# YangChenApril/AMContrast3D

Measured on AMD Instinct MI355X. Metric: train-step points/sec (fwd+bwd) on 24k-pt S3DIS clouds, higher is better.
Workload: dtype f32; 1 GPU; PointNeXt-S + AMContrast3D-AA, S3DIS-shaped 24000-pt voxelised (0.04 m) clouds, batch 8/GPU, fwd + CE/contrast loss + bwd + clip + AdamW; global_batch=8, points=24000, parallelism=dp1, launch=hipGraph replay, batches_per_joint_fps_launch=4, geometry_queue_cus=176, feature_graph_segments=1, collectives=none, update=captured in the feature graph

## Files before the change

amcontrast3d_amd/_lib.py:

```python
import ctypes
import os
import subprocess

_CSRC = os.path.join(os.path.dirname(os.path.abspath(__file__)), "csrc")
_SO = os.environ.get("AMC3D_LIB") or os.path.join(_CSRC, "libamc3d_hip.so")

_vp, _i, _f, _sz, _l = ctypes.c_void_p, ctypes.c_int, ctypes.c_float, ctypes.c_size_t, ctypes.c_long
_ll = ctypes.c_longlong

SIGNATURES = {
    "amc3d_version": (ctypes.c_char_p, []),
    "amc3d_last_error": (ctypes.c_char_p, []),
    "amc3d_stream_create_dedicated": (_i, [ctypes.POINTER(ctypes.c_void_p)]),
    "amc3d_stream_create_masked": (_i, [_vp, _i, _i]),
    "amc3d_reserve_scratch": (_i, [_i, _vp, _vp]),
    "amc3d_stream_destroy": (_i, [_vp]),
    "amc3d_grid_search_workspace_bytes": (_sz, [_i, _i, _i]),
    "amc3d_grid_search_pays": (_i, [_i, _i, _i]),
    "amc3d_ball_query": (_i, [_i, _i, _i, _f, _i, _vp, _vp, _vp, _vp, _sz, _vp]),
    "amc3d_group_points": (_i, [_i, _i, _i, _i, _i, _vp, _vp, _vp, _vp]),
    "amc3d_group_points_grad": (_i, [_i, _i, _i, _i, _i, _vp, _vp, _vp, _vp, _sz, _vp]),
    "amc3d_gather_points": (_i, [_i, _i, _i, _i, _vp, _vp, _vp, _vp]),
    "amc3d_gather_points_grad": (_i, [_i, _i, _i, _i, _vp, _vp, _vp, _vp]),
    "amc3d_fps_workspace_bytes": (_sz, [_i, _i]),
    "amc3d_furthest_point_sampling": (_i, [_i, _i, _i, _vp, _vp, _vp, _vp, _sz, _vp]),
    "amc3d_three_nn": (_i, [_i, _i, _i, _vp, _vp, _vp, _vp, _vp, _sz, _vp]),
    "amc3d_three_interpolate": (_i, [_i, _i, _i, _i, _vp, _vp, _vp, _vp, _vp]),
    "amc3d_three_interpolate_add": (_i, [_i, _i, _i, _i, _vp, _vp, _vp, _vp, _vp, _vp]),
    "amc3d_three_interpolate_grad": (_i, [_i, _i, _i, _i, _vp, _vp, _vp, _vp, _vp, _sz, _vp]),
    "amc3d_three_interpolate_grad_route": (_i, [_i, _i, _i, _i, ctypes.POINTER(_i), ctypes.POINTER(_i)]),
    "amc3d_three_interpolate_grad_write": (_i, [_i, _i, _i, _i, _vp, _vp, _vp, _vp, _vp]),
    "amc3d_three_interpolate_grad_lds": (_i, [_i, _i, _i, _i, _i, _i, _i, _vp, _vp, _vp, _vp, _vp]),
    "amc3d_knnquery_workspace_bytes": (_sz, [_i, _i, _i, _i]),
    "amc3d_knnquery_uses_grid": (_i, [_i, _i, _i, _i]),
    "amc3d_knnquery": (_i, [_i, _i, _i, _i, _vp, _vp, _vp, _vp, _vp, _vp, _vp, _sz, _i, _vp]),
    "amc3d_knn_batch_workspace_bytes": (_sz, [_i, _i, _i, _i]),
    "amc3d_knn_batch": (_i, [_i, _i, _i, _i, _i, _vp, _vp, _vp, _vp, _i, _vp, _sz, _i, _vp]),
    "amc3d_knn_group_dp": (_i, [_i, _i, _i, _i, _vp, _vp, _vp, _i, _i, _vp, _vp, _vp]),
    "amc3d_pointops_ballquery": (_i, [_i, _f, _i, _i, _i, _vp, _vp, _vp, _vp, _vp, _vp]),
    "amc3d_pointops_furthestsampling": (_i, [_i, _i, _i, _vp, _vp, _vp, _vp, _vp, _vp]),
    "amc3d_pointops_grouping_forward": (_i, [_i, _i, _i, _i, _vp, _vp, _vp, _vp]),
    "amc3d_pointops_grouping_backward": (_i, [_i, _i, _i, _i, _vp, _vp, _vp, _vp]),
    "amc3d_pointops_interpolation_forward": (_i, [_i, _i, _i, _i, _i, _vp, _vp, _vp, _vp, _vp]),
    "amc3d_pointops_interpolation_backward": (_i, [_i, _i, _i, _i, _vp, _vp, _vp, _vp, _vp]),
    "amc3d_pointops_subtraction_forward": (_i, [_i, _i, _i, _vp, _vp, _vp, _vp, _vp]),
    "amc3d_pointops_subtraction_backward": (_i, [_i, _i, _i, _vp, _vp, _vp, _vp, _vp]),
    "amc3d_pointops_aggregation_forward": (_i, [_i, _i, _i, _i, _i, _vp, _vp, _vp, _vp, _vp, _vp]),
    "amc3d_pointops_aggregation_backward": (_i, [_i, _i, _i, _i, _vp, _vp, _vp, _vp, _vp, _vp, _vp, _vp, _vp]),
    "amc3d_pointops_scatter_csr": (_i, [_i, _i, _i, _i, _i, _vp, _vp, _vp, _vp, _vp, _vp]),
    "amc3d_vote_labels": (_i, [_i, _i, _i, _vp, _vp, _vp, _vp]),
    "amc3d_posmask": (_i, [_i, _i, _i, _vp, _vp, _vp, _vp]),
    "amc3d_ambiguity_workspace_bytes": (_sz, [_i]),
    "amc3d_ambiguity": (_i, [_i, _i, _i, _i, _f, _vp, _vp, _vp, _vp, _vp, _sz, _vp]),
    "amc3d_contrast_csr_workspace_bytes": (_sz, [_i]),
    "amc3d_contrast_csr": (_i, [_i, _i, _i, _vp, _vp, _vp, _vp, _sz, _vp]),
    "amc3d_contrast_backward_csr_supported": (_i, [_i]),
    "amc3d_contrast_backward_rows_supported": (_i, [_i]),
    "amc3d_contrast_backward_csr": (_i, [_i, _i, _i, _i, _vp, _vp, _vp, _vp, _vp, _vp, _vp, _f, _f, _f, _vp, _vp, _vp, _vp,
                                         _vp, _vp]),
    "amc3d_contrast_mutual_workspace_bytes": (_sz, [_i]),
    "amc3d_contrast_mutual": (_i, [_i, _i, _i, _vp, _vp, _vp, _vp, _vp, _vp, _sz, _vp]),
    "amc3d_contrast_backward_mutual_workspace_bytes": (_sz, [_i]),
    "amc3d_contrast_backward_mutual": (_i, [_i, _i, _i, _i, _vp, _vp, _vp, _vp, _vp, _vp, _vp, _f, _f, _f, _vp, _vp, _vp, _vp, _vp, _sz,
                                            _vp, _vp]),
    "amc3d_contrast_stages_forward_cm": (_i, [_i, _vp, _f, _f, _f, _f, _vp, _vp]),
    "amc3d_contrast_stages_backward_cm_workspace_bytes": (_sz, [_i, _vp]),
    "amc3d_contrast_stages_backward_cm": (_i, [_i, _vp, _f, _f, _f, _f, _vp, _vp, _sz, _vp]),
    "amc3d_contrast_variant_forward": (_i, [_i, _i, _i, _i, _vp, _vp, _vp, _vp, _vp, _i, _i, _i, _i, _f, _f, _f, _vp, _vp, _vp, _vp,
                                            _vp, _vp]),
    "amc3d_contrast_variant_backward": (_i, [_i, _i, _i, _i, _vp, _vp, _vp, _vp, _vp, _vp, _vp, _i, _i, _i, _i, _f, _f, _f, _vp, _vp,
                                             _vp, _vp, _vp, _vp]),
    "amc3d_adamw_chunk": (_i, []),
    "amc3d_adamw_step": (_i, [_vp, _vp, _i, ctypes.c_double, ctypes.c_double, _f, _f, _vp, _vp, _vp]),
    "amc3d_select_anchors_ints": (_sz, [_i]),
    "amc3d_select_anchors": (_i, [_i, _vp, _vp, _sz, _vp]),
    "amc3d_contrast_forward": (_i, [_i, _i, _i, _i, _vp, _vp, _vp, _vp, _vp, _f, _f, _f, _vp, _vp, _vp, _vp, _vp, _vp, _vp]),
# ... 112 lines not shown
    "amc3d_grouped_conv_bn_backward_csr": (_i, [_i] * 6 + [_vp, _i] + [_vp] * 16 + [_i, _vp, _vp, _vp, _sz, _vp]),
    "amc3d_grouped_conv_bn_backward_csr_strided": (_i, [_i] * 6 + [_vp, _i] + [_vp] * 6 + [_l] + [_vp] * 8 + [_l] + [_vp] * 2 + [_i, _vp, _vp, _vp, _sz, _vp]),
    "amc3d_group_csr_dp": (_i, [_i, _i, _i, _vp, _vp, _vp, _vp]),
    "amc3d_sa_tail_supported": (_i, [_i, _i, _i]),
    "amc3d_sa_tail_pays": (_i, [_i, _i]),
    "amc3d_sa_tail_workspace_bytes": (_sz, [_i, _i, _i, _i]),
    "amc3d_sa_tail_forward": (_i, [_i, _i, _i, _i, _i] + [_vp] * 8 + [_f, _f, _i] + [_vp] * 10 + [_sz, _vp]),
    "amc3d_sa_tail_backward": (_i, [_i, _i, _i, _i, _i] + [_vp] * 10 + [_i, _vp, _vp, _vp, _vp, _i] + [_vp] * 5 + [_sz, _vp]),
    "amc3d_bn_workspace_bytes": (_sz, [_i]),
    "amc3d_bn_stats": (_i, [_i, _i, _l, _f, _vp, _vp, _vp, _vp, _vp, _sz, _vp]),
    "amc3d_bn_forward": (_i, [_i, _i, _l, _i, _i, _f, _f, _vp, _vp, _vp, _vp, _vp, _vp, _vp, _vp, _vp, _vp, _vp, _vp, _sz, _vp]),
    "amc3d_bn_update_running": (_i, [_i, _f, _vp, _vp, _vp, _vp, _vp, _vp]),
    "amc3d_bn_act": (_i, [_i, _i, _l, _i, _vp, _vp, _vp, _vp, _vp, _vp, _vp]),
    "amc3d_bn_max": (_i, [_i, _i, _i, _i, _i, _vp, _vp, _vp, _vp, _vp, _vp, _vp, _vp]),
    "amc3d_bn_backward": (_i, [_i, _i, _l, _i, _i, _vp, _vp, _vp, _vp, _vp, _vp, _vp, _vp, _vp, _vp, _vp, _sz, _vp]),
    "amc3d_bn_sums": (_i, [_i, _i, _l, _vp, _vp, _vp, _sz, _vp]),
    "amc3d_bn_forward_synced": (_i, [_i, _i, _l, _i, _i, _f, _f, _vp, _vp, _vp, _vp, _vp, _vp, _vp, _vp, _vp, _vp, _vp, _vp, _vp]),
    "amc3d_bn_backward_sums": (_i, [_i, _i, _l, _i, _i, _vp, _vp, _vp, _vp, _vp, _vp, _vp, _vp, _vp, _vp, _vp, _sz, _vp]),
    "amc3d_bn_backward_synced": (_i, [_i, _i, _l, _i, _i, _vp, _vp, _vp, _vp, _vp, _vp, _vp, _vp, _vp, _vp, _vp]),
}


CONTRAST_MAX_STAGES = 8


class ContrastStageDesc(ctypes.Structure):
    _fields_ = ([(n, _i) for n in ("b", "C", "n", "k", "nbr_stride")]
                + [(n, _vp) for n in ("f_cm", "nbr", "posmask", "a", "sel", "mutual", "rev", "norm", "unit", "stats", "loss_pt",
                                      "mean_cnt", "rec", "grad_cm")])


def build(force=False):
    cmd = ["make", "-C", _CSRC, "-j8"] + (["-B"] if force else [])
    proc = subprocess.run(cmd, stdout=subprocess.PIPE, stderr=subprocess.STDOUT, text=True)
    if proc.returncode != 0:
        raise RuntimeError("building libamc3d_hip.so failed:\n" + proc.stdout)
    return _SO


_lib = None


def load():
    global _lib
    if _lib is not None:
        return _lib
# ... 18 lines not shown
```

amcontrast3d_amd/csrc/knn.hip:

```cpp

#include "common.h"

namespace amc {

constexpr int KNN_TILE = 1024;
constexpr int KNN_WAVES = 16;
constexpr int KNN_MAXK = 100;

__device__ __forceinline__ void reheap(float *dist, int *idx, int k)
{
    int root = 0;
    int child = 1;
    while (child < k) {
        if (child + 1 < k && dist[child + 1] > dist[child]) child++;
        if (dist[root] > dist[child]) return;
        const float tf = dist[root]; dist[root] = dist[child]; dist[child] = tf;
        const int ti = idx[root]; idx[root] = idx[child]; idx[child] = ti;
        root = child;
        child = root * 2 + 1;
    }
}

__global__ __launch_bounds__(KNN_WAVES * 64) void knn_exact_kernel(
    int m, int nsample, int nbatch, const float *__restrict__ xyz, const float *__restrict__ new_xyz,
// ... 932 lines not shown
        }
#ifdef AMC_KNN_DIAG
        if (threadIdx.x == 0)
            printf("replay q=%d T=%d |S|=%d steps=%d survsteps=%d surv=%d acc=%d  prefix_clk=%lld surv_clk=%lld\n", pt, end, ns,
                   n_steps, n_survsteps, n_surv, n_acc, (long long)(clock64() - t_a), t_surv);
#endif
        if (wave == 0) {
            float root = s_root;
            for (int r = nsample; r < ns; ++r) {
                const float cd = s_rd[r];
                if (cd < root) {
                    lh_replace_root(hp, nsample, lane, cd, s_ri[r]);
                    root = lh_root(hp);
                }
            }
            for (int i = nsample - 1; i > 0; i--) {
                const float d0 = lh_root(hp), di = __int_as_float(__builtin_amdgcn_readlane(__float_as_int(hp.d), i));
                const int j0 = __builtin_amdgcn_readlane(hp.id, 0), ji = __builtin_amdgcn_readlane(hp.id, i);
                if (lane == i) { hp.d = d0; hp.id = j0; }
                lh_replace_root(hp, i, lane, di, ji);
            }
            if (lane < nsample) {
                idx[(size_t)pt * nsample + lane] = hp.id;
                dist2[(size_t)pt * nsample + lane] = hp.d;
            }
        }
    }
}

static int kg_build(const KnnWorkspace &w, char *base, int n, int m, int nbatch, const float *xyz, const float *new_xyz,
                    const int *offset, const int *new_offset, int ksample, int sub, float hscale, float fixed_h,
                    hipStream_t stream)
{
    GridParams *gp = (GridParams *)(base + w.params);
    int *bbox = (int *)(base + w.bbox);
    float *samples = (float *)(base + w.samples);
    int *fb_count = (int *)(base + w.fb_count);
    int *cell_start = (int *)(base + w.cell_start);
    int *cursor = (int *)(base + w.cursor);
    float4 *sorted = (float4 *)(base + w.sorted);
    const size_t cells = (size_t)knn_cell_cap(n) + 1;
    if (int st = fill_i32(cell_start, 0, (size_t)(cursor - cell_start) + cells, stream)) return st;
    hipLaunchKernelGGL(kg_init_kernel, dim3(1), dim3(64), 0, stream, bbox, fb_count);
    hipLaunchKernelGGL(kg_bbox_kernel, dim3(min(div_up(n, 256), 64)), dim3(256), 0, stream, n, xyz, bbox);
    if (!(fixed_h > 0.f))
        hipLaunchKernelGGL(kg_sample_kernel, dim3(KG_SAMPLES), dim3(1024), 0, stream, m, ksample, nbatch, sub, xyz, new_xyz,
                           offset, new_offset, samples);
    hipLaunchKernelGGL(kg_params_kernel, dim3(1), dim3(64), 0, stream, n, nbatch, hscale, fixed_h, bbox, samples, gp);
    hipLaunchKernelGGL(kg_count_kernel, dim3(div_up(n, 256)), dim3(256), 0, stream, n, nbatch, xyz, offset, gp,
// ... 260 lines not shown
    if (nsample <= KGG_MAXK) {
        constexpr int per_wg = 4 * (64 / KGG_MAXK);
        hipLaunchKernelGGL(kg_query_group_kernel<KGG_MAXK>, dim3(min(div_up(m, per_wg), 256 * 32)), dim3(256), 0, stream, m,
                           nsample, nbatch, self, new_xyz, offset, new_offset, gp, cell_start, sorted, idx, dist2, fb_list,
                           fb_count);
    } else {
        hipLaunchKernelGGL(kg_query_kernel, dim3(min(div_up(m, 4), 256 * 32)), dim3(256), 0, stream, m, nsample, nbatch, self,
                           new_xyz, offset, new_offset, gp, cell_start, sorted, idx, dist2, fb_list, fb_count);
    }
    hipLaunchKernelGGL(knn_exact_list_kernel, dim3(256), dim3(1024), 0, stream, nsample, nbatch, xyz, new_xyz, offset,
                       new_offset, idx, dist2, (const int *)fb_list, (const int *)fb_count, (const GridParams *)gp,
                       (const int *)cell_start, (const float4 *)sorted);
    return launch_status("amc3d_knnquery");
}

AMC_API int amc3d_knnquery(int m, int nsample, int n, int nbatch, const float *xyz, const float *new_xyz,
                           const int *offset, const int *new_offset, int *idx, float *dist2, void *workspace,
                           size_t workspace_bytes, int reuse_grid, void *stream_)
{
    return knn_search(m, nsample, n, nbatch, xyz, new_xyz, offset, new_offset, idx, dist2, workspace, workspace_bytes,
                      reuse_grid, stream_);
}

namespace amc {

constexpr int KB_QT = 64;

struct KnnBatchWorkspace {
    size_t grid_bytes, off_s, off_q, idx, dist2, total;
};

static KnnBatchWorkspace knn_batch_layout(int b, int n, int m, int ksearch)
{
    KnnBatchWorkspace w;
    w.grid_bytes = knn_layout(b * n, b * m).total;
    w.off_s = w.grid_bytes;
    w.off_q = align256(w.off_s + (size_t)b * 4);
    w.idx = align256(w.off_q + (size_t)b * 4);
    w.dist2 = align256(w.idx + (size_t)b * m * ksearch * 4);
    w.total = align256(w.dist2 + (size_t)b * m * ksearch * 4);
    return w;
}

__global__ __launch_bounds__(256) void knn_batch_epilogue_kernel(int n, int m, int ksearch, int dilation, int kout,
                                                                 const int *__restrict__ raw_idx,
                                                                 const float *__restrict__ raw_d2, int *__restrict__ idx,
// ... 73 lines not shown
```

amcontrast3d_amd/csrc/loss.hip:

```cpp
#include "common.h"

#include <type_traits>
#include <utility>

namespace amc {

__global__ __launch_bounds__(256) void vote_labels_kernel(int m, int kr, int ncls, const int *__restrict__ labels0,
                                                          const int *__restrict__ nbr, int *__restrict__ out)
{
    const int lane = threadIdx.x & 63;
    const int q = blockIdx.x * 4 + (threadIdx.x >> 6);
    if (q >= m) return;
    int c0 = -1, c1 = -1;
    if (lane < kr) c0 = labels0[nbr[(size_t)q * kr + lane]];
    if (lane + 64 < kr) c1 = labels0[nbr[(size_t)q * kr + lane + 64]];
    int best = -1, bestc = 0;
    for (int c = 0; c < ncls; ++c) {
        const int cnt = (int)__popcll(__ballot(c0 == c)) + (int)__popcll(__ballot(c1 == c));
        if (cnt > best) { best = cnt; bestc = c; }
    }
    if (lane == 0) out[q] = bestc;
}

__global__ void posmask_kernel(int m, int k, int nbr_stride, const int *__restrict__ labels,
// ... 10 lines not shown
                                                              const unsigned char *__restrict__ posmask,
                                                              const int *__restrict__ nbr, int *__restrict__ n_pos,
                                                              float *__restrict__ d_pos, float *__restrict__ d_neg,
                                                              int *__restrict__ max_npos)
{
    const int i = blockIdx.x * blockDim.x + threadIdx.x;
    int np = 0;
    if (i < m) {
        const float px = p[(size_t)i * 3], py = p[(size_t)i * 3 + 1], pz = p[(size_t)i * 3 + 2];
        const float ss = __fadd_rn(__fadd_rn(__fmul_rn(px, px), __fmul_rn(py, py)), __fmul_rn(pz, pz));
        float dp = 0.f, dn = 0.f;
        for (int j = 0; j < k; ++j) {
            const int nb = nbr[(size_t)i * nbr_stride + j];
            const float qx = p[(size_t)nb * 3], qy = p[(size_t)nb * 3 + 1], qz = p[(size_t)nb * 3 + 2];
            const float dot = __fadd_rn(__fadd_rn(__fmul_rn(px, qx), __fmul_rn(py, qy)), __fmul_rn(pz, qz));
            const float sd = __fadd_rn(__fadd_rn(__fmul_rn(qx, qx), __fmul_rn(qy, qy)), __fmul_rn(qz, qz));
            float dd = __fadd_rn(__fadd_rn(__fmul_rn(-2.f, dot), ss), sd);
            if (mode == 3) dd = sqrtf(__fadd_rn(fabsf(dd), 1e-12f));
            const bool pos = posmask[(size_t)i * k + j] != 0;
            np += pos ? 1 : 0;
            dp = __fadd_rn(dp, pos ? dd : 0.f);
            dn = __fadd_rn(dn, pos ? 0.f : dd);
        }
        n_pos[i] = np;
        d_pos[i] = mode == 1 ? 5.f : dp;
        d_neg[i] = mode == 1 ? 5.f : dn;
    }
    int w = np;
    for (int s = 32; s >= 1; s >>= 1) w = max(w, __shfl_xor(w, s, 64));
    if ((threadIdx.x & 63) == 0 && w > 0) atomicMax(max_npos, w);
}

__global__ void ambiguity_kernel(int m, int k, float beta, const int *__restrict__ n_pos,
                                 const float *__restrict__ d_pos, const float *__restrict__ d_neg,
                                 const int *__restrict__ max_npos, float *__restrict__ a)
{
    const int i = blockIdx.x * blockDim.x + threadIdx.x;
    if (i >= m) return;
    const int top = *max_npos;
    const int np = n_pos[i];
    float v = __fdiv_rn((float)abs(np - top), (float)top);
    if (0 < np && np < top) {
        const float cc = __fsub_rn(__fdiv_rn((float)np, d_pos[i]), __fdiv_rn((float)(k - np), d_neg[i]));
        v = __fdiv_rn(1.f, __fadd_rn(1.f, powf(2.718281828459045f, __fmul_rn(beta, cc))));
    }
    a[i] = v;
// ... 1525 lines not shown
AMC_API size_t amc3d_ambiguity_workspace_bytes(int m) { return (size_t)m * 12 + 64; }

AMC_API int amc3d_ambiguity(int m, int k, int nbr_stride, int mode, float beta, const float *p,
                            const unsigned char *posmask, const int *nbr, float *a, void *workspace,
                            size_t workspace_bytes, void *stream_)
{
    if (m <= 0) return 0;
    if (k <= 0 || nbr_stride < k || mode < 1 || mode > 3 || !p || !posmask || !nbr || !a || !workspace ||
        workspace_bytes < amc3d_ambiguity_workspace_bytes(m))
        return bad_arg("amc3d_ambiguity: bad argument");
    hipStream_t stream = (hipStream_t)stream_;
    int *max_npos = (int *)workspace;
    int *n_pos = (int *)((char *)workspace + 64);
    float *d_pos = (float *)(n_pos + m);
    float *d_neg = d_pos + m;
    if (int st = fill_i32(max_npos, 0, 1, stream)) return st;
    hipLaunchKernelGGL(ambiguity_stats_kernel, dim3(div_up(m, 256)), dim3(256), 0, stream, m, k, nbr_stride, mode, p,
                       posmask, nbr, n_pos, d_pos, d_neg, max_npos);
    hipLaunchKernelGGL(ambiguity_kernel, dim3(div_up(m, 256)), dim3(256), 0, stream, m, k, beta, n_pos, d_pos, d_neg,
                       max_npos, a);
    return launch_status("amc3d_ambiguity");
}

AMC_API size_t amc3d_select_anchors_ints(int m) { return (size_t)(m > 0 ? m : 0) + 1 + (size_t)div_up(m > 0 ? m : 1, 256); }

AMC_API int amc3d_select_anchors(int m, const float *a, int *sel, size_t sel_ints, void *stream_)
{
    if (m < 0 || !sel || sel_ints < amc3d_select_anchors_ints(m) || (m > 0 && !a))
        return bad_arg("amc3d_select_anchors: bad argument");
    hipStream_t stream = (hipStream_t)stream_;
    if (m == 0) return fill_i32(sel, 0, 1, stream);
    const int nb = div_up(m, 256);
    hipLaunchKernelGGL(select_count_kernel, dim3(nb), dim3(256), 0, stream, m, a, sel);
    hipLaunchKernelGGL(select_write_kernel, dim3(nb), dim3(256), 0, stream, m, a, sel);
    return launch_status("amc3d_select_anchors");
}


template <class F>
static bool with_lpr(int C, F &&fn)
{
    switch (C) {
    case 16: fn(int_c<4>{}); return true;
    case 32: fn(int_c<8>{}); return true;
    case 64: fn(int_c<16>{}); return true;
    case 128: fn(int_c<32>{}); return true;
// ... 557 lines not shown
```

amcontrast3d_amd/openpoints/AMContrast3D/AEF/utils.py:

```python
import torch
import torch.nn.functional as F

from openpoints.cpp.pointops.functions import pointops


def get_subscene_label_CBL(stage_n, stage_i, stage_list, target, nstride, num_classes, ignore_index):
    if ignore_index is not None:
        num_classes = num_classes + 1
        if (target == ignore_index).sum() > 0:
            target = target.clone()
            target[target == ignore_index] = num_classes - 1
    x = F.one_hot(target, num_classes)
    if stage_i == 0:
        return x.float()
    kr = int(torch.prod(nstride[:stage_i]))
    src = stage_list['up'][0]
    dst = stage_list[stage_n][stage_i]
    neighbor_idx, _ = pointops.knnquery(kr, src['p_out'], dst['p_out'], src['offset'], dst['offset'])
    neighbor_idx = neighbor_idx.view(-1).long()
    x = x[neighbor_idx, :].view(dst['p_out'].shape[0], kr, x.shape[1])
    return x.float().mean(-2)


def get_subscene_class(stage_n, stage_i, stage_list, target, nstride, num_classes, ignore_index):
    from amcontrast3d_amd import ops
    if ignore_index is not None:
        num_classes = num_classes + 1
        target = torch.where(target == ignore_index, torch.full_like(target, num_classes - 1), target)
    labels0 = target.to(torch.int32)
    if stage_i == 0:
        return labels0, num_classes
    kr = int(torch.prod(nstride[:stage_i]))
    src = stage_list['up'][0]
    dst = stage_list[stage_n][stage_i]
    knn = ops.knnquery_squared if labels0.is_cuda else pointops.knnquery
    neighbor_idx, _ = knn(kr, src['p_out'], dst['p_out'], src['offset'], dst['offset'])
    return ops.vote_labels(labels0, neighbor_idx, num_classes), num_classes


def fetch_pxo(stage_n, stage_i, stage_list, ftype):
    stage = stage_list[stage_n][stage_i]
    return stage['p_out'], stage['f_out'], stage['offset']


def get_ftype(ftype):
    if ftype in ['out', 'fout', 'f_out', 'latent', 'logits', 'probs']:
        ptype = 'p_out'
        ftype = 'f_out' if ftype in ['out', 'fout'] else ftype
    elif ftype in ['sample', 'fsample', 'f_sample']:
        ptype = 'p_sample'
        ftype = 'f_sample' if ftype in ['sample', 'fsample'] else ftype
    else:
        raise KeyError(f'not supported ftype = {ftype}')
    return ftype, ptype
```

amcontrast3d_amd/openpoints/AMContrast3D/MarginContrast.py:

```python
import os

import torch
import torch.nn as nn
import torch.nn.functional as F

from openpoints.cpp.pointops.functions import pointops
from .AEF.ambiguity import ambiguity_function
from .AEF.function import _eps
from .AEF.utils import fetch_pxo, get_ftype, get_subscene_class, get_subscene_label_CBL


def _posmask_cnt(labels, neighbor_label):
    return torch.argmax(torch.unsqueeze(labels, -2), -1) == torch.argmax(neighbor_label, -1)


def plan_stage(n, i, stageACE_list, target, nstride, num_classes, ignore_index, ambiguity_args, ftype='f_out'):
    from amcontrast3d_amd import ops
    p, o = stageACE_list[n][i]['p_out'], stageACE_list[n][i]['offset']
    labels, _ = get_subscene_class(n, i, stageACE_list, target, nstride, num_classes, ignore_index)
    knn = ops.knnquery_squared if p.is_cuda else pointops.knnquery
    neighbor_idx, neighbor_d2 = knn(ambiguity_args.nsample, p, p, o, o)
    neighbor_idx = neighbor_idx[..., 1:]
    posmask = ops.posmask_from_labels(labels, neighbor_idx)
    a, shares = ambiguity_function(p, posmask, neighbor_idx.shape[1], neighbor_idx, ambiguity_args.cctype,
                                   ambiguity_args.ccbeta, ambiguity_args.vis, ambiguity_args.nu)
    anchors = ops.select_anchors(a) if a.is_cuda and a.dtype == torch.float32 else None
    rev = mutual = None
    default_form = ops.contrast_form_is_default(getattr(ambiguity_args, 'margin', 'adaptive'), getattr(ambiguity_args, 'db', '-m'),
                                                getattr(ambiguity_args, 'supervisedCL', 'Method1'),
                                                getattr(ambiguity_args, 'temperature', 1.0))
    if anchors is not None and neighbor_idx.shape[1] <= 64 and not default_form:
        rev = ops.contrast_csr(neighbor_idx, anchors)
    elif anchors is not None and neighbor_idx.shape[1] <= 64:
        d2 = neighbor_d2[..., 1:] if (torch.is_tensor(neighbor_d2) and neighbor_d2.dtype == torch.float32 and o.numel() == 1
                                      and neighbor_d2.shape[0] == neighbor_idx.shape[0] > neighbor_idx.shape[1] + 2) else None
        mutual, rev = ops.contrast_mutual(neighbor_idx, a, d2)
    return {'neighbor_idx': neighbor_idx, 'posmask': posmask, 'ambiguity': a, 'shares': shares, 'anchors': anchors,
            'rev': rev, 'mutual': mutual}


def _stage_plan(n, i, stageACE_list, target, nstride, num_classes, ignore_index, ambiguity_args, ftype):
    geometry = stageACE_list.get('geometry') if hasattr(stageACE_list, 'get') else None
    if geometry is not None and 'loss' in geometry:
        return geometry['loss'][i]
    return plan_stage(n, i, stageACE_list, target, nstride, num_classes, ignore_index, ambiguity_args, ftype)


class AmbiguityHead(nn.Module):
# ... 169 lines not shown
```

amcontrast3d_amd/ops.py:

```python
import ctypes

import torch
from torch.autograd import Function

from . import _lib, timing


def _ptr(t):
    return ctypes.c_void_p(t.data_ptr())


_dedicated = []


def _destroy_dedicated():
    if not _dedicated:
        return
    try:
        torch.cuda.synchronize()
        for handle, _ in _dedicated:
            _lib.load().amc3d_stream_destroy(handle)
    finally:
        _dedicated.clear()

# ... 411 lines not shown
            new_xyz = xyz
        assert xyz.is_contiguous() and new_xyz.is_contiguous()
        _need_gpu(xyz, new_xyz, offset, new_offset)
        _need_dtype(torch.float32, xyz=xyz, new_xyz=new_xyz)
        _need_dtype(torch.int32, offset=offset, new_offset=new_offset)
        nsample = int(nsample)
        n, m, nb = xyz.shape[0], new_xyz.shape[0], offset.shape[0]
        idx = torch.empty(m, nsample, dtype=torch.int32, device=xyz.device)
        dist2 = torch.empty(m, nsample, dtype=torch.float32, device=xyz.device)
        lib = _lib.load()
        wbytes = int(lib.amc3d_knnquery_workspace_bytes(n, m, nsample, nb))
        offset, new_offset = offset.contiguous(), new_offset.contiguous()
        key = (xyz.data_ptr(), n, offset.data_ptr(), nb, _stream(xyz).value)
        cached = _grid_cache.get(key) if _grid_cache is not None else None
        gridded = bool(lib.amc3d_knnquery_uses_grid(m, nsample, n, nb))
        reuse = gridded and cached is not None and cached.numel() >= wbytes
        work = cached if reuse else torch.empty(wbytes, dtype=torch.uint8, device=xyz.device)
        if _grid_cache is not None and gridded and not reuse:
            _grid_cache[key] = work
        with torch.cuda.device(xyz.device), timing.span("knnquery", (n + m) * 12 + m * nsample * 8):
            _lib.check(lib.amc3d_knnquery(m, nsample, n, nb, _ptr(xyz), _ptr(new_xyz), _ptr(offset),
                                          _ptr(new_offset), _ptr(idx), _ptr(dist2), _ptr(work), work.numel(),
                                          int(reuse), _stream(xyz)), "knnquery")
        ctx.mark_non_differentiable(idx)
        if _knn_squared:
            return idx, dist2
        return idx, torch.sqrt(dist2)

    @staticmethod
    def backward(ctx, a=None, b=None):
        return None, None, None, None, None


knnquery = KNNQuery.apply
_knn_squared = False


def knnquery_squared(nsample, xyz, new_xyz, offset, new_offset):
    global _knn_squared
    prev, _knn_squared = _knn_squared, True
    try:
        return KNNQuery.apply(nsample, xyz, new_xyz, offset, new_offset)
    finally:
        _knn_squared = prev


KNN_BATCH_MAX = 100
_KNN_DIST_LAYOUT = {"bmk": 0, "bkm": 1}


@torch.no_grad()
def knn_batch(k, support, query=None, dilation=1, dist=None):
    if query is None:
        query = support
    assert support.is_contiguous() and query.is_contiguous()
    _need_gpu(support, query)
    _need_dtype(torch.float32, support=support, query=query)
    if support.dim() != 3 or query.dim() != 3 or support.shape[2] != 3 or query.shape[2] != 3 or support.shape[0] != query.shape[0]:
        raise RuntimeError(f"knn_batch: expected (B,N,3) and (B,M,3), got {tuple(support.shape)} and {tuple(query.shape)}")
    k, dilation = int(k), int(dilation)
    ksearch = k * dilation
    B, N, _ = support.shape
    M = query.shape[1]
    if k <= 0 or dilation <= 0 or ksearch > KNN_BATCH_MAX:
        raise RuntimeError(f"knn_batch: k * dilation must be in 1..{KNN_BATCH_MAX}, got {k} * {dilation}")
    if ksearch > N:
        raise RuntimeError(f"knn_batch: k * dilation = {ksearch} out of range for {N} support points")
# ... 56 lines not shown
    _need_gpu(labels0, neighbor_idx)
    assert labels0.dtype == torch.int32 and neighbor_idx.dtype == torch.int32 and neighbor_idx.is_contiguous()
    m, kr = neighbor_idx.shape
    out = torch.empty(m, dtype=torch.int32, device=labels0.device)
    with torch.cuda.device(labels0.device), timing.span("vote_labels", m * kr * 8 + m * 4):
        _lib.check(_lib.load().amc3d_vote_labels(m, kr, int(num_classes), _ptr(labels0), _ptr(neighbor_idx), _ptr(out),
                                                 _stream(labels0)), "vote_labels")
    return out


def posmask_from_labels(labels, neighbor_idx):
    _need_gpu(labels, neighbor_idx)
    nptr, k, stride, keep = _nbr_view(neighbor_idx)
    m = labels.shape[0]
    out = torch.empty(m, k, dtype=torch.bool, device=labels.device)
    with torch.cuda.device(labels.device), timing.span("posmask", m * k * 9 + m * 4):
        _lib.check(_lib.load().amc3d_posmask(m, k, stride, _ptr(labels), nptr, _ptr(out), _stream(labels)), "posmask")
    return out


_CCTYPE = {"Method1": 1, "Method2": 2, "Method3": 3}


def ambiguity(p, posmask, neighbor_idx, cctype, beta):
    _need_gpu(p, posmask, neighbor_idx)
    assert p.is_contiguous() and posmask.is_contiguous() and posmask.dtype == torch.bool
    nptr, k, stride, keep = _nbr_view(neighbor_idx)
    m = p.shape[0]
    lib = _lib.load()
    wbytes = int(lib.amc3d_ambiguity_workspace_bytes(m))
    work = torch.empty(wbytes, dtype=torch.uint8, device=p.device)
    a = torch.empty(m, dtype=torch.float32, device=p.device)
    with torch.cuda.device(p.device), timing.span("ambiguity", m * (12 + 4) + m * k * (4 + 1), moved=m * (12 + 4) + m * k * (4 + 1 + 12)):
        _lib.check(lib.amc3d_ambiguity(m, k, stride, _CCTYPE[cctype], float(beta), _ptr(p), _ptr(posmask), nptr,
                                       _ptr(a), _ptr(work), wbytes, _stream(p)), "ambiguity")
    return a


def select_anchors(a):
    _need_gpu(a)
    _need_dtype(torch.float32, a=a)
    assert a.is_contiguous() and a.dim() == 1
    m = a.shape[0]
    lib = _lib.load()
    n = int(lib.amc3d_select_anchors_ints(m))
    sel = torch.empty(n, dtype=torch.int32, device=a.device)
# ... 1801 lines not shown
```

include/amc3d.h:

```cpp
#ifndef AMC3D_H
#define AMC3D_H

#include <stddef.h>
#include <stdint.h>

#ifdef __cplusplus
extern "C" {
#endif

const char *amc3d_version(void);
const char *amc3d_last_error(void);

int amc3d_stream_create_dedicated(void **stream);
int amc3d_stream_create_masked(void **stream, int first_cu, int n_cus);
int amc3d_reserve_scratch(int bytes_per_lane, int *scratch_out, void *stream);
int amc3d_stream_destroy(void *stream);


size_t amc3d_grid_search_workspace_bytes(int b, int n_support, int m_queries);
int amc3d_grid_search_pays(int b, int n_support, int m_queries);
int amc3d_ball_query(int b, int n, int m, float radius, int nsample,
                     const float *new_xyz, const float *xyz, int *idx,
                     void *workspace, size_t workspace_bytes, void *stream);

// ... 20 lines not shown
int amc3d_three_interpolate(int b, int c, int m, int n, const float *points,
                            const int *idx, const float *weight, float *out, void *stream);

int amc3d_three_interpolate_add(int b, int c, int m, int n, const float *points, const int *idx, const float *weight,
                                const float *base, float *out, void *stream);
int amc3d_three_interpolate_grad(int b, int c, int n, int m, const float *grad_out,
                                 const int *idx, const float *weight, float *grad_points,
                                 void *workspace, size_t workspace_bytes, void *stream);
int amc3d_three_interpolate_grad_route(int b, int c, int n, int m, int *cg, int *threads);
int amc3d_three_interpolate_grad_write(int b, int c, int n, int m, const float *grad_out, const int *idx,
                                       const float *weight, float *grad_points, void *stream);
int amc3d_three_interpolate_grad_lds(int b, int c, int n, int m, int cg, int threads, int accumulate, const float *grad_out,
                                     const int *idx, const float *weight, float *grad_points, void *stream);
int amc3d_three_interpolate_grad_csr(int b, int c, int n, int m, const float *grad_out, const int *idx, const float *weight,
                                     const int *rev_start, const int *rev_edge, float *grad_points, void *stream);


size_t amc3d_knnquery_workspace_bytes(int n, int m, int nsample, int nbatch);
int amc3d_knnquery_uses_grid(int m, int nsample, int n, int nbatch);
int amc3d_knnquery(int m, int nsample, int n, int nbatch, const float *xyz, const float *new_xyz,
                   const int *offset, const int *new_offset, int *idx, float *dist2,
                   void *workspace, size_t workspace_bytes, int reuse_grid, void *stream);

#define AMC_KNN_DIST_BMK 0
#define AMC_KNN_DIST_BKM 1
size_t amc3d_knn_batch_workspace_bytes(int b, int n, int m, int ksearch);
int amc3d_knn_batch(int b, int n, int m, int ksearch, int dilation, const float *support, const float *query,
                    int *idx, float *dist, int dist_layout, void *workspace, size_t workspace_bytes,
                    int reuse_grid, void *stream);

int amc3d_knn_group_dp(int b, int n, int m, int k, const float *support, const float *query, const int *idx,
                       int relative, int normalize, float *dp, float *cloud_max, void *stream);


int amc3d_pointops_ballquery(int m, float radius, int nsample, int n, int nbatch, const float *xyz, const float *new_xyz,
                             const int *offset, const int *new_offset, int *idx, void *stream);

int amc3d_pointops_furthestsampling(int nbatch, int n_max, int n, const float *xyz, const int *offset,
                                    const int *new_offset, float *tmp, int *idx, void *stream);

int amc3d_pointops_grouping_forward(int m, int nsample, int c, int n, const float *input, const int *idx, float *output,
                                    void *stream);
int amc3d_pointops_grouping_backward(int m, int nsample, int c, int n, const float *grad_output, const int *idx,
                                     float *grad_input, void *stream);

int amc3d_pointops_interpolation_forward(int n, int c, int k, int m, int accumulate, const float *input, const int *idx,
// ... 7 lines not shown
                                        float *grad_input1, float *grad_input2, void *stream);

int amc3d_pointops_aggregation_forward(int n, int nsample, int c, int w_c, int accumulate, const float *input,
                                       const float *position, const float *weight, const int *idx, float *output,
                                       void *stream);
int amc3d_pointops_aggregation_backward(int n, int nsample, int c, int w_c, const float *input, const float *position,
                                        const float *weight, const int *idx, const float *grad_output, float *grad_input,
                                        float *grad_position, float *grad_weight, void *stream);

int amc3d_pointops_scatter_csr(int kind, int n_targets, int c, int per, int w_c, const float *g, const float *w,
                               const int *rev_start, const int *rev_edge, float *out, void *stream);


int amc3d_vote_labels(int m, int kr, int num_classes, const int *labels0, const int *nbr_idx, int *labels,
                      void *stream);

int amc3d_posmask(int m, int k, int nbr_stride, const int *labels, const int *nbr, unsigned char *posmask,
                  void *stream);

size_t amc3d_ambiguity_workspace_bytes(int m);
int amc3d_ambiguity(int m, int k, int nbr_stride, int mode, float beta, const float *p,
                    const unsigned char *posmask, const int *nbr, float *a, void *workspace,
                    size_t workspace_bytes, void *stream);

size_t amc3d_select_anchors_ints(int m);
int amc3d_select_anchors(int m, const float *a, int *sel, size_t sel_ints, void *stream);

int amc3d_contrast_forward(int m, int C, int k, int nbr_stride, const float *f, const int *nbr,
                           const unsigned char *posmask, const float *a, const int *sel, float mu, float nu,
                           float temperature, float *norm, float *unit, float *sim, float *stats, float *loss_pt,
                           float *mean_cnt, void *stream);

int amc3d_contrast_forward_cm(int b, int C, int n, int k, int nbr_stride, const float *f_cm, const int *nbr,
                              const unsigned char *posmask, const float *a, const int *sel, float mu, float nu,
                              float temperature, float *norm, float *unit, float *sim, float *stats, float *loss_pt,
                              float *mean_cnt, void *stream);

int amc3d_contrast_backward(int m, int C, int k, int nbr_stride, const float *f, const float *norm,
                            const int *nbr, const unsigned char *posmask, const float *a, const int *sel, float mu,
                            float nu, float temperature, const float *sim, const float *mean_cnt,
                            const float *grad_out, float *grad_f, void *stream);

size_t amc3d_contrast_csr_workspace_bytes(int m);
int amc3d_contrast_csr(int m, int k, int nbr_stride, const int *nbr, const int *sel, int *rev, void *workspace,
                       size_t workspace_bytes, void *stream);
int amc3d_contrast_backward_csr_supported(int C);
// ... 437 lines not shown
```

Measured before the change: 35.16 million points/s.

## Reuse cached kNN rows for label-vote queries and fuse posmask with ambiguity

Label voting now takes its kNN from a cached self-kNN of the support cloud. Each query is matched to its identical support point through the grid, the first kr columns of that point's cached row are copied, and any query that cannot be matched exactly falls back to the exact per-query search. A separate fused loss_rows kernel computes the positive mask, neighbour distances and per-point sums in one LDS-staged pass, followed by the ambiguity kernel. This removes a full grid kNN search per stage and one kernel pass over the neighbour lists, at the cost of extra caching state and an approximate-match path that must fall back correctly.

```diff
diff --git a/amcontrast3d_amd/_lib.py b/amcontrast3d_amd/_lib.py
--- a/amcontrast3d_amd/_lib.py
+++ b/amcontrast3d_amd/_lib.py
@@ -34,6 +34,7 @@
     "amc3d_knnquery_workspace_bytes": (_sz, [_i, _i, _i, _i]),
     "amc3d_knnquery_uses_grid": (_i, [_i, _i, _i, _i]),
     "amc3d_knnquery": (_i, [_i, _i, _i, _i, _vp, _vp, _vp, _vp, _vp, _vp, _vp, _sz, _i, _vp]),
+    "amc3d_knn_prefix": (_i, [_i, _i, _i, _i, _vp, _vp, _vp, _vp, _i, _i, _vp, _vp, _vp, _vp, _vp, _sz, _i, _vp]),
     "amc3d_knn_batch_workspace_bytes": (_sz, [_i, _i, _i, _i]),
     "amc3d_knn_batch": (_i, [_i, _i, _i, _i, _i, _vp, _vp, _vp, _vp, _i, _vp, _sz, _i, _vp]),
     "amc3d_knn_group_dp": (_i, [_i, _i, _i, _i, _vp, _vp, _vp, _i, _i, _vp, _vp, _vp]),
@@ -52,6 +53,8 @@
     "amc3d_posmask": (_i, [_i, _i, _i, _vp, _vp, _vp, _vp]),
     "amc3d_ambiguity_workspace_bytes": (_sz, [_i]),
     "amc3d_ambiguity": (_i, [_i, _i, _i, _i, _f, _vp, _vp, _vp, _vp, _vp, _sz, _vp]),
+    "amc3d_loss_rows_supported": (_i, [_i]),
+    "amc3d_loss_rows": (_i, [_i, _i, _i, _i, _f, _vp, _vp, _vp, _vp, _vp, _vp, _sz, _vp]),
     "amc3d_contrast_csr_workspace_bytes": (_sz, [_i]),
     "amc3d_contrast_csr": (_i, [_i, _i, _i, _vp, _vp, _vp, _vp, _sz, _vp]),
     "amc3d_contrast_backward_csr_supported": (_i, [_i]),
@@ -210,6 +213,7 @@
 
 
 CONTRAST_MAX_STAGES = 8
+KNN_FALLBACK_COUNT_OFFSET = 1024
 
 
 class ContrastStageDesc(ctypes.Structure):
diff --git a/amcontrast3d_amd/csrc/knn.hip b/amcontrast3d_amd/csrc/knn.hip
--- a/amcontrast3d_amd/csrc/knn.hip
+++ b/amcontrast3d_amd/csrc/knn.hip
@@ -978,9 +978,56 @@
             }
             if (lane < nsample) {
                 idx[(size_t)pt * nsample + lane] = hp.id;
-                dist2[(size_t)pt * nsample + lane] = hp.d;
-            }
-        }
+                if (dist2) dist2[(size_t)pt * nsample + lane] = hp.d;
+            }
+        }
+    }
+}
+
+__global__ __launch_bounds__(256) void kg_prefix_kernel(int m, int kr, int nb, int row_stride, const float *__restrict__ new_xyz,
+                                                        const int *__restrict__ new_offset, const GridParams *__restrict__ gp,
+                                                        const int *__restrict__ cell_start, const float4 *__restrict__ sorted,
+                                                        const int *__restrict__ rows_idx, const float *__restrict__ rows_d2,
+                                                        int *__restrict__ idx, float *__restrict__ dist2,
+                                                        int *__restrict__ fb_list, int *__restrict__ fb_count)
+{
+    const int lane = threadIdx.x & 63, gl = lane & 31;
+    const long qg = ((long)blockIdx.x * 256 + threadIdx.x) >> 5;
+    const bool act = qg < m;
+    const int q = act ? (int)qg : 0;
+    const GridParams g = *gp;
+    const int seg = nb > 1 ? seg_of(q, new_offset, nb) : 0;
+    const float qx = new_xyz[(size_t)q * 3], qy = new_xyz[(size_t)q * 3 + 1], qz = new_xyz[(size_t)q * 3 + 2];
+    const int cx = cell_coord(qx, g.minx, g.inv_h, g.nx), cy = cell_coord(qy, g.miny, g.inv_h, g.ny),
+              cz = cell_coord(qz, g.minz, g.inv_h, g.nz);
+    const size_t cell = (size_t)seg * g.ncell + ((size_t)cz * g.ny + cy) * g.nx + cx;
+    const int b = cell_start[cell];
+    const int len = act ? cell_start[cell + 1] - b : 0;
+    const int wave_len = max(len, __shfl_xor(len, 32, 64));
+    int found = 0, cnt = 0;
+    for (int c0 = 0; c0 < wave_len; c0 += 32) {
+        const int c = c0 + gl;
+        const bool valid = c < len;
+        const float4 pt = sorted[valid ? b + c : 0];
+        const bool match = valid && pt.x == qx && pt.y == qy && pt.z == qz;
+        const unsigned bits = grp_bits<32>(__ballot(match), lane);
+        cnt += (int)__popc(bits);
+        const int v = __shfl(__float_as_int(pt.w), (lane & 32) + (bits ? (int)__builtin_ctz(bits) : 0), 64);
+        if (bits) found = v;
+    }
+    const bool one = act && cnt == 1;
+    const size_t row = one ? (size_t)found * row_stride : 0;
+    const float d = gl <= kr ? rows_d2[row + gl] : 0.f;
+    const float dnext = __shfl_down(d, 1, 64);
+    const bool bad = (gl < kr && !(d < dnext)) || (gl == kr && !(d < 1e10f));
+    const bool use = one && grp_bits<32>(__ballot(bad), lane) == 0;
+    if (use) {
+        if (gl < kr) {
+            idx[(size_t)q * kr + gl] = rows_idx[row + gl];
+            if (dist2) dist2[(size_t)q * kr + gl] = d;
+        }
+    } else if (act && gl == 0) {
+        fb_list[atomicAdd(fb_count, 1)] = q;
     }
 }
 
@@ -1287,6 +1334,37 @@
                       reuse_grid, stream_);
 }
 
+AMC_API int amc3d_knn_prefix(int m, int kr, int n, int nbatch, const float *xyz, const float *new_xyz, const int *offset,
+                             const int *new_offset, int k0, int row_stride, const int *rows_idx, const float *rows_d2,
+                             int *idx, float *dist2, void *workspace, size_t workspace_bytes, int reuse_grid, void *stream_)
+{
+    if (m <= 0) return 0;
+    if (kr <= 0 || kr >= k0 || kr >= 32 || row_stride < k0 || nbatch <= 0 || nbatch > 64 || n <= 0 || !xyz || !new_xyz ||
+        !offset || !new_offset || !rows_idx || !rows_d2 || !idx)
+        return bad_arg("amc3d_knn_prefix: bad argument (0 < kr < k0 <= row_stride, kr <= 31, nbatch <= 64)");
+    if (!reuse_grid && n < 4 * KG_SAMPLES) return bad_arg("amc3d_knn_prefix: too few support points to build a grid");
+    hipStream_t stream = (hipStream_t)stream_;
+    const KnnWorkspace w = knn_layout(n, m);
+    if (!workspace || workspace_bytes < w.total) return bad_arg("amc3d_knn_prefix: workspace too small");
+    char *base = (char *)workspace;
+    static_assert(AMC_KNN_FALLBACK_COUNT_OFFSET == 1024, "knn_layout: fb_count");
+    if (reuse_grid) {
+        hipLaunchKernelGGL(kg_init_kernel, dim3(1), dim3(64), 0, stream, (int *)(base + w.bbox), (int *)(base + w.fb_count));
+    } else if (int st = kg_build(w, base, n, m, nbatch, xyz, new_xyz, offset, new_offset, (kr + 3) / 4, 4, 0.7f, 0.f, stream)) {
+        return st;
+    }
+    const GridParams *gp = (const GridParams *)(base + w.params);
+    int *fb_count = (int *)(base + w.fb_count);
+    const int *cell_start = (const int *)(base + w.cell_start);
+    const float4 *sorted = (const float4 *)(base + w.sorted);
+    int *fb_list = (int *)(base + w.fb_list);
+    hipLaunchKernelGGL(kg_prefix_kernel, dim3(div_up((long)m * 32, 256)), dim3(256), 0, stream, m, kr, nbatch, row_stride, new_xyz,
+                       new_offset, gp, cell_start, sorted, rows_idx, rows_d2, idx, dist2, fb_list, fb_count);
+    hipLaunchKernelGGL(knn_exact_list_kernel, dim3(256), dim3(1024), 0, stream, kr, nbatch, xyz, new_xyz, offset, new_offset,
+                       idx, dist2, (const int *)fb_list, (const int *)fb_count, gp, cell_start, sorted);
+    return launch_status("amc3d_knn_prefix");
+}
+
 namespace amc {
 
 constexpr int KB_QT = 64;
diff --git a/amcontrast3d_amd/csrc/loss.hip b/amcontrast3d_amd/csrc/loss.hip
--- a/amcontrast3d_amd/csrc/loss.hip
+++ b/amcontrast3d_amd/csrc/loss.hip
@@ -56,6 +56,73 @@
             dp = __fadd_rn(dp, pos ? dd : 0.f);
             dn = __fadd_rn(dn, pos ? 0.f : dd);
         }
+        n_pos[i] = np;
+        d_pos[i] = mode == 1 ? 5.f : dp;
+        d_neg[i] = mode == 1 ? 5.f : dn;
+    }
+    int w = np;
+    for (int s = 32; s >= 1; s >>= 1) w = max(w, __shfl_xor(w, s, 64));
+    if ((threadIdx.x & 63) == 0 && w > 0) atomicMax(max_npos, w);
+}
+
+constexpr int LR_PTS = 128;
+
+__global__ __launch_bounds__(256) void loss_rows_kernel(int m, int k, int nbr_stride, int mode, const int *__restrict__ labels,
+                                                        const float *__restrict__ p, const int *__restrict__ nbr,
+                                                        unsigned char *__restrict__ posmask, int *__restrict__ n_pos,
+                                                        float *__restrict__ d_pos, float *__restrict__ d_neg,
+                                                        int *__restrict__ max_npos)
+{
+    extern __shared__ float lr_lds[];
+    float *s_dd = lr_lds;
+    float *s_pt = s_dd + LR_PTS * k;
+    int *s_lab = (int *)(s_pt + LR_PTS * 4);
+    unsigned char *s_pm = (unsigned char *)(s_lab + LR_PTS);
+    const int i0 = blockIdx.x * LR_PTS;
+    const int npts = min(LR_PTS, m - i0);
+    if ((int)threadIdx.x < npts) {
+        const size_t i = (size_t)i0 + threadIdx.x;
+        const float px = p[i * 3], py = p[i * 3 + 1], pz = p[i * 3 + 2];
+        s_pt[threadIdx.x * 4] = px;
+        s_pt[threadIdx.x * 4 + 1] = py;
+        s_pt[threadIdx.x * 4 + 2] = pz;
+        s_pt[threadIdx.x * 4 + 3] = __fadd_rn(__fadd_rn(__fmul_rn(px, px), __fmul_rn(py, py)), __fmul_rn(pz, pz));
+        s_lab[threadIdx.x] = labels[i];
+    }
+    __syncthreads();
+    const int nedge = npts * k;
+    for (int e = threadIdx.x; e < nedge; e += 256) {
+        const int il = e / k, j = e - il * k;
+        const int nb = nbr[((size_t)i0 + il) * nbr_stride + j];
+        const bool pos = labels[nb] == s_lab[il];
+        float dd = 0.f;
+        if (mode != 1) {
+            const float px = s_pt[il * 4], py = s_pt[il * 4 + 1], pz = s_pt[il * 4 + 2], ss = s_pt[il * 4 + 3];
+            const float qx = p[(size_t)nb * 3], qy = p[(size_t)nb * 3 + 1], qz = p[(size_t)nb * 3 + 2];
+            const float dot = __fadd_rn(__fadd_rn(__fmul_rn(px, qx), __fmul_rn(py, qy)), __fmul_rn(pz, qz));
+            const float sd = __fadd_rn(__fadd_rn(__fmul_rn(qx, qx), __fmul_rn(qy, qy)), __fmul_rn(qz, qz));
+            dd = __fadd_rn(__fadd_rn(__fmul_rn(-2.f, dot), ss), sd);
+            if (mode == 3) dd = sqrtf(__fadd_rn(fabsf(dd), 1e-12f));
+        }
+        posmask[(size_t)i0 * k + e] = pos ? 1 : 0;
+        s_dd[e] = dd;
+        s_pm[e] = pos ? 1 : 0;
+    }
+    __syncthreads();
+    if (threadIdx.x >= LR_PTS) return;
+    int np = 0;
+    if ((int)threadIdx.x < npts) {
+        const float *dd_i = s_dd + threadIdx.x * k;
+        const unsigned char *pm_i = s_pm + threadIdx.x * k;
+        float dp = 0.f, dn = 0.f;
+        for (int j = 0; j < k; ++j) {
+            const float dd = dd_i[j];
+            const bool pos = pm_i[j] != 0;
+            np += pos ? 1 : 0;
+            dp = __fadd_rn(dp, pos ? dd : 0.f);
+            dn = __fadd_rn(dn, pos ? 0.f : dd);
+        }
+        const size_t i = (size_t)i0 + threadIdx.x;
         n_pos[i] = np;
         d_pos[i] = mode == 1 ? 5.f : dp;
         d_neg[i] = mode == 1 ? 5.f : dn;
@@ -1627,6 +1694,31 @@
     return launch_status("amc3d_ambiguity");
 }
 
+AMC_API int amc3d_loss_rows_supported(int k) { return (k >= 1 && k <= 64) ? 1 : 0; }
+
+AMC_API int amc3d_loss_rows(int m, int k, int nbr_stride, int mode, float beta, const int *labels, const float *p,
+                            const int *nbr, unsigned char *posmask, float *a, void *workspace, size_t workspace_bytes,
+                            void *stream_)
+{
+    if (m <= 0) return 0;
+    if (!amc3d_loss_rows_supported(k) || nbr_stride < k || mode < 1 || mode > 3 || !labels || !p || !nbr || !posmask ||
+        !workspace || workspace_bytes < amc3d_ambiguity_workspace_bytes(m))
+        return bad_arg("amc3d_loss_rows: bad argument (k must be in 1..64)");
+    hipStream_t stream = (hipStream_t)stream_;
+    int *max_npos = (int *)workspace;
+    int *n_pos = (int *)((char *)workspace + 64);
+    float *d_pos = (float *)(n_pos + m);
+    float *d_neg = d_pos + m;
+    if (int st = fill_i32(max_npos, 0, 1, stream)) return st;
+    const size_t lds = (size_t)LR_PTS * (5 * (size_t)k + 20);
+    hipLaunchKernelGGL(loss_rows_kernel, dim3(div_up(m, LR_PTS)), dim3(256), lds, stream, m, k, nbr_stride, mode, labels, p,
+                       nbr, posmask, n_pos, d_pos, d_neg, max_npos);
+    if (a)
+        hipLaunchKernelGGL(ambiguity_kernel, dim3(div_up(m, 256)), dim3(256), 0, stream, m, k, beta, n_pos, d_pos, d_neg,
+                           max_npos, a);
+    return launch_status("amc3d_loss_rows");
+}
+
 AMC_API size_t amc3d_select_anchors_ints(int m) { return (size_t)(m > 0 ? m : 0) + 1 + (size_t)div_up(m > 0 ? m : 1, 256); }
 
 AMC_API int amc3d_select_anchors(int m, const float *a, int *sel, size_t sel_ints, void *stream_)
diff --git a/amcontrast3d_amd/openpoints/AMContrast3D/AEF/utils.py b/amcontrast3d_amd/openpoints/AMContrast3D/AEF/utils.py
--- a/amcontrast3d_amd/openpoints/AMContrast3D/AEF/utils.py
+++ b/amcontrast3d_amd/openpoints/AMContrast3D/AEF/utils.py
@@ -33,8 +33,10 @@
     kr = int(torch.prod(nstride[:stage_i]))
     src = stage_list['up'][0]
     dst = stage_list[stage_n][stage_i]
-    knn = ops.knnquery_squared if labels0.is_cuda else pointops.knnquery
-    neighbor_idx, _ = knn(kr, src['p_out'], dst['p_out'], src['offset'], dst['offset'])
+    if labels0.is_cuda:
+        neighbor_idx = ops.knn_of_support_points(kr, src['p_out'], dst['p_out'], src['offset'], dst['offset'])
+    else:
+        neighbor_idx, _ = pointops.knnquery(kr, src['p_out'], dst['p_out'], src['offset'], dst['offset'])
     return ops.vote_labels(labels0, neighbor_idx, num_classes), num_classes
 
 
diff --git a/amcontrast3d_amd/openpoints/AMContrast3D/MarginContrast.py b/amcontrast3d_amd/openpoints/AMContrast3D/MarginContrast.py
--- a/amcontrast3d_amd/openpoints/AMContrast3D/MarginContrast.py
+++ b/amcontrast3d_amd/openpoints/AMContrast3D/MarginContrast.py
@@ -5,7 +5,7 @@
 import torch.nn.functional as F
 
 from openpoints.cpp.pointops.functions import pointops
-from .AEF.ambiguity import ambiguity_function
+from .AEF.ambiguity import _LazyShares, ambiguity_function
 from .AEF.function import _eps
 from .AEF.utils import fetch_pxo, get_ftype, get_subscene_class, get_subscene_label_CBL
 
@@ -21,9 +21,14 @@
     knn = ops.knnquery_squared if p.is_cuda else pointops.knnquery
     neighbor_idx, neighbor_d2 = knn(ambiguity_args.nsample, p, p, o, o)
     neighbor_idx = neighbor_idx[..., 1:]
-    posmask = ops.posmask_from_labels(labels, neighbor_idx)
-    a, shares = ambiguity_function(p, posmask, neighbor_idx.shape[1], neighbor_idx, ambiguity_args.cctype,
-                                   ambiguity_args.ccbeta, ambiguity_args.vis, ambiguity_args.nu)
+    if (not ambiguity_args.vis and ambiguity_args.cctype in ('Method1', 'Method2', 'Method3')
+            and ops.loss_rows_supported(p, labels, neighbor_idx)):
+        posmask, a = ops.posmask_and_ambiguity(labels, p.contiguous(), neighbor_idx, ambiguity_args.cctype, ambiguity_args.ccbeta)
+        shares = _LazyShares(a, ambiguity_args.nu)
+    else:
+        posmask = ops.posmask_from_labels(labels, neighbor_idx)
+        a, shares = ambiguity_function(p, posmask, neighbor_idx.shape[1], neighbor_idx, ambiguity_args.cctype,
+                                       ambiguity_args.ccbeta, ambiguity_args.vis, ambiguity_args.nu)
     anchors = ops.select_anchors(a) if a.is_cuda and a.dtype == torch.float32 else None
     rev = mutual = None
     default_form = ops.contrast_form_is_default(getattr(ambiguity_args, 'margin', 'adaptive'), getattr(ambiguity_args, 'db', '-m'),
diff --git a/amcontrast3d_amd/ops.py b/amcontrast3d_amd/ops.py
--- a/amcontrast3d_amd/ops.py
+++ b/amcontrast3d_amd/ops.py
@@ -457,6 +457,8 @@
             _lib.check(lib.amc3d_knnquery(m, nsample, n, nb, _ptr(xyz), _ptr(new_xyz), _ptr(offset),
                                           _ptr(new_offset), _ptr(idx), _ptr(dist2), _ptr(work), work.numel(),
                                           int(reuse), _stream(xyz)), "knnquery")
+        if _grid_cache is not None and gridded and m == n and new_xyz.data_ptr() == xyz.data_ptr() and new_offset.data_ptr() == offset.data_ptr():
+            _grid_cache[("rows",) + key] = (idx, dist2)
         ctx.mark_non_differentiable(idx)
         if _knn_squared:
             return idx, dist2
@@ -478,6 +480,52 @@
         return KNNQuery.apply(nsample, xyz, new_xyz, offset, new_offset)
     finally:
         _knn_squared = prev
+
+
+KNN_PREFIX_MAX = 31
+
+
+@torch.no_grad()
+def knn_prefix(kr, xyz, new_xyz, offset, new_offset, rows_idx, rows_d2, work=None, want_dist=True):
+    assert xyz.is_contiguous() and new_xyz.is_contiguous() and rows_idx.is_contiguous() and rows_d2.is_contiguous()
+    _need_gpu(xyz, new_xyz, offset, new_offset, rows_idx, rows_d2)
+    _need_dtype(torch.float32, xyz=xyz, new_xyz=new_xyz, rows_d2=rows_d2)
+    _need_dtype(torch.int32, offset=offset, new_offset=new_offset, rows_idx=rows_idx)
+    kr = int(kr)
+    n, m, nb = xyz.shape[0], new_xyz.shape[0], offset.shape[0]
+    k0 = rows_idx.shape[1]
+    if rows_idx.shape != (n, k0) or rows_d2.shape != (n, k0) or not 0 < kr < k0 or kr > KNN_PREFIX_MAX:
+        raise RuntimeError(f"knn_prefix: rows {tuple(rows_idx.shape)} / {tuple(rows_d2.shape)} for {n} support points, kr = {kr}")
+    lib = _lib.load()
+    wbytes = int(lib.amc3d_knnquery_workspace_bytes(n, m, kr, nb))
+    offset, new_offset = offset.contiguous(), new_offset.contiguous()
+    if work is None and _grid_cache is not None:
+        kept = _grid_cache.get((xyz.data_ptr(), n, offset.data_ptr(), nb, _stream(xyz).value))
+        work = kept if kept is not None and kept.numel() >= wbytes else None
+    reuse = work is not None
+    if reuse and work.numel() < wbytes:
+        raise RuntimeError("knn_prefix: the kept workspace is too small for these queries")
+    if not reuse:
+        work = torch.empty(wbytes, dtype=torch.uint8, device=xyz.device)
+    idx = torch.empty(m, kr, dtype=torch.int32, device=xyz.device)
+    dist2 = torch.empty(m, kr, dtype=torch.float32, device=xyz.device) if want_dist else None
+    with torch.cuda.device(xyz.device), timing.span("knn_prefix", m * (12 + (kr + 1) * 4 + kr * (12 if want_dist else 8))):
+        _lib.check(lib.amc3d_knn_prefix(m, kr, n, nb, _ptr(xyz), _ptr(new_xyz), _ptr(offset), _ptr(new_offset), k0,
+                                        rows_idx.stride(0), _ptr(rows_idx), _ptr(rows_d2), _ptr(idx),
+                                        _ptr(dist2) if want_dist else None, _ptr(work), work.numel(), int(reuse),
+                                        _stream(xyz)), "knn_prefix")
+    count = work[_lib.KNN_FALLBACK_COUNT_OFFSET:_lib.KNN_FALLBACK_COUNT_OFFSET + 4].view(torch.int32)
+    return idx, dist2, count
+
+
+def knn_of_support_points(kr, xyz, new_xyz, offset, new_offset):
+    key = (xyz.data_ptr(), xyz.shape[0], offset.data_ptr(), offset.shape[0], _stream(xyz).value)
+    rows = _grid_cache.get(("rows",) + key) if _grid_cache is not None and offset.is_contiguous() else None
+    work = _grid_cache.get(key) if rows is not None else None
+    if (work is not None and kr <= KNN_PREFIX_MAX and kr < rows[0].shape[1] and offset.shape[0] <= 64 and new_xyz.dtype == torch.float32
+            and work.numel() >= int(_lib.load().amc3d_knnquery_workspace_bytes(xyz.shape[0], new_xyz.shape[0], kr, offset.shape[0]))):
+        return knn_prefix(kr, xyz, new_xyz, offset, new_offset, rows[0], rows[1], work=work, want_dist=False)[0]
+    return knnquery_squared(kr, xyz, new_xyz, offset, new_offset)[0]
 
 
 KNN_BATCH_MAX = 100
@@ -580,6 +628,32 @@
 _CCTYPE = {"Method1": 1, "Method2": 2, "Method3": 3}
 
 
+def loss_rows_supported(p, labels, neighbor_idx):
+    return (p.is_cuda and p.dtype == torch.float32 and labels.dtype == torch.int32 and neighbor_idx.dtype == torch.int32
+            and bool(_lib.load().amc3d_loss_rows_supported(neighbor_idx.shape[1])))
+
+
+def posmask_and_ambiguity(labels, p, neighbor_idx, cctype, beta, stats=False):
+    _need_gpu(labels, p, neighbor_idx)
+    _need_dtype(torch.float32, p=p)
+    _need_dtype(torch.int32, labels=labels)
+    assert p.is_contiguous() and labels.is_contiguous()
+    nptr, k, stride, keep = _nbr_view(neighbor_idx)
+    m = p.shape[0]
+    lib = _lib.load()
+    wbytes = int(lib.amc3d_ambiguity_workspace_bytes(m))
+    work = torch.empty(wbytes, dtype=torch.uint8, device=p.device)
+    posmask = torch.empty(m, k, dtype=torch.bool, device=p.device)
+    a = torch.empty(m, dtype=torch.float32, device=p.device)
+    with torch.cuda.device(p.device), timing.span("loss_rows", m * (12 + 4 + 4) + m * k * (4 + 1), moved=m * 20 + m * k * (4 + 1 + 4 + 12)):
+        _lib.check(lib.amc3d_loss_rows(m, k, stride, _CCTYPE[cctype], float(beta), _ptr(labels), _ptr(p), nptr, _ptr(posmask),
+                                       _ptr(a), _ptr(work), wbytes, _stream(p)), "loss_rows")
+    if not stats:
+        return posmask, a
+    return posmask, a, (work[:4].view(torch.int32), work[64:64 + 4 * m].view(torch.int32),
+                        work[64 + 4 * m:64 + 8 * m].view(torch.float32), work[64 + 8 * m:64 + 12 * m].view(torch.float32))
+
+
 def ambiguity(p, posmask, neighbor_idx, cctype, beta):
     _need_gpu(p, posmask, neighbor_idx)
     assert p.is_contiguous() and posmask.is_contiguous() and posmask.dtype == torch.bool
diff --git a/include/amc3d.h b/include/amc3d.h
--- a/include/amc3d.h
+++ b/include/amc3d.h
@@ -66,6 +66,11 @@
                    const int *offset, const int *new_offset, int *idx, float *dist2,
                    void *workspace, size_t workspace_bytes, int reuse_grid, void *stream);
 
+#define AMC_KNN_FALLBACK_COUNT_OFFSET 1024
+int amc3d_knn_prefix(int m, int kr, int n, int nbatch, const float *xyz, const float *new_xyz, const int *offset,
+                     const int *new_offset, int k0, int row_stride, const int *rows_idx, const float *rows_d2, int *idx,
+                     float *dist2, void *workspace, size_t workspace_bytes, int reuse_grid, void *stream);
+
 #define AMC_KNN_DIST_BMK 0
 #define AMC_KNN_DIST_BKM 1
 size_t amc3d_knn_batch_workspace_bytes(int b, int n, int m, int ksearch);
@@ -119,6 +124,11 @@
 int amc3d_ambiguity(int m, int k, int nbr_stride, int mode, float beta, const float *p,
                     const unsigned char *posmask, const int *nbr, float *a, void *workspace,
                     size_t workspace_bytes, void *stream);
+
+int amc3d_loss_rows_supported(int k);
+int amc3d_loss_rows(int m, int k, int nbr_stride, int mode, float beta, const int *labels, const float *p,
+                    const int *nbr, unsigned char *posmask, float *a, void *workspace, size_t workspace_bytes,
+                    void *stream);
 
 size_t amc3d_select_anchors_ints(int m);
 int amc3d_select_anchors(int m, const float *a, int *sel, size_t sel_ints, void *stream);
```

Result: faster. 35.61 million points/s (median of 6 runs) (+1.3%).
